# xingyizhou/CenterNet

Hardware: AMD Instinct MI355X
Metric: images/sec whole-node, 512x512 ctdet (higher is better)
Workload: dtype f32s; 1 GPU; ctdet resdcn_18 512x512, batch 32 per GPU (BASELINE configs[1]), network + fused sigmoid/peak-NMS/top-K decode, K=100; global_batch=32, parallelism=image-sharded x1

## Files before the change

centernet_amd/csrc/cn_heads_at.hip:

```cpp
#include "cn_common.h"
#include "cn_internal.h"

namespace {

constexpr int HA_NT = 256;
constexpr int HA_CELLS = 16;
constexpr int HA_CC = 64;
constexpr int HA_ROW = 9 * HA_CC;
constexpr int HA_MAXN = 768;
constexpr int HA_MAXJ = 17;
constexpr int HA_MAXOUT = 2 + 2 * HA_MAXJ + 2;
enum { HA_CTDET = 0, HA_POSE = 1, HA_DDD = 2 };
constexpr int HA_PF = 4;
constexpr int HA_MAXGROUPS = 5;
constexpr int HA_GROUP_HEADS = 3;
constexpr int HA_DDD_OUT = 16;

struct HeadsAtGroup {
    const cn_f32x4 *w1;
    const float *b1, *w2, *b2;
    int n_heads;
    int cout[HA_GROUP_HEADS];
    int col[HA_GROUP_HEADS];
    int voff[HA_GROUP_HEADS];
};

struct HeadsAtArgs {
    const char *feat;
    const float *scores;
    const int32_t *inds, *clses;
    const cn_f32x4 *w1;
    const float *b1;
    const float *w2;
    const float *b2;
    float *dets;
    float *vals;
    float mul;
    int H, W, Cin, pitch, K, hidden, n_heads, N;
    int c0, c1;
    int out;
    int J;
    HeadsAtGroup grp[HA_MAXGROUPS];
    int D;
    int vals_out;
    int raw_depth;
    int half_group;
};

__device__ __forceinline__ void ha_ctdet_row(const HeadsAtArgs &a, size_t row, int ind, const float *o)
{
    float *d = a.dets + row * 6;
    const float score = a.scores[row];
    const float cls = (float)a.clses[row];
    if (ind < 0) {
        const float nan = __builtin_nanf("");
        d[0] = nan; d[1] = nan; d[2] = nan; d[3] = nan; d[4] = score; d[5] = cls;
        if (a.vals)
            for (int v = 0; v < a.out; ++v) a.vals[row * a.out + v] = nan;
        return;
    }
    const int yi = ind / a.W, xi = ind - yi * a.W;
    float xs = (float)xi, ys = (float)yi;
    if (a.n_heads > 1) {
        xs = xs + o[2];
        ys = ys + o[3];
    } else {
        xs = xs + 0.5f;
        ys = ys + 0.5f;
    }
    const float w = o[0];
    const float h = o[1];
    d[0] = xs - w / 2;
    d[1] = ys - h / 2;
    d[2] = xs + w / 2;
    d[3] = ys + h / 2;
    d[4] = score;
    d[5] = cls;
    if (a.vals)
        for (int v = 0; v < a.out; ++v) a.vals[row * a.out + v] = o[v];
}

__device__ __forceinline__ float ha_pose_col(const HeadsAtArgs &a, size_t row, int ind, const float *o, int col)
{
    const int D = 5 + 2 * a.J + 1;
    if (col == 4) return a.scores[row];
    if (col == D - 1) return (float)a.clses[row];
    if (ind < 0) return __builtin_nanf("");
    const int yi = ind / a.W, xi = ind - yi * a.W;
    if (col >= 5) {
        const int v = col - 5;
        return o[2 + v] + (float)((v & 1) ? yi : xi);
    }
    const bool isy = col & 1;
    float c = (float)(isy ? yi : xi);
    if (a.n_heads > 2) c = c + o[2 + 2 * a.J + (isy ? 1 : 0)];
    else c = c + 0.5f;
    const float half = o[isy ? 1 : 0] / 2;
    return col < 2 ? c - half : c + half;
}

template <bool F32S, int CT, int NS, int TASK = HA_CTDET>
__global__ __launch_bounds__(HA_NT) void decode_heads_at_cells_kernel(const HeadsAtArgs a)
{
    constexpr int CG = HA_CELLS / CT;
    constexpr int TPC = HA_NT / CG;
    static_assert(TPC % 64 == 0, "the lanes of a wave read one cell's patch");
    constexpr int HROW = NS * TPC > HA_ROW ? NS * TPC : HA_ROW;
    static_assert(NS * TPC <= HA_MAXN && HA_CELLS * HROW * 4 <= 48 * 1024, "static LDS");
    __shared__ __attribute__((aligned(16))) float lds[HA_CELLS * HROW];
    __shared__ int s_ind[HA_CELLS];
    __shared__ float s_out[HA_CELLS * (TASK == HA_POSE ? HA_MAXOUT : TASK == HA_DDD ? HA_DDD_OUT : 4)];

    const int tid = threadIdx.x;
    const int b = blockIdx.y;
    const int k0 = blockIdx.x * HA_CELLS;
    const int ncell = min(HA_CELLS, a.K - k0);
    const int HW = a.H * a.W;
    int N = a.N, out = a.out, hc0 = a.c0, hc1 = a.c1;
    const cn_f32x4 *w1 = a.w1;
    const float *b1 = a.b1, *w2 = a.w2, *b2 = a.b2;
    if constexpr (TASK == HA_DDD) {
        const HeadsAtGroup &g = a.grp[blockIdx.z];
        N = g.n_heads * a.hidden;
        hc0 = g.cout[0];
        hc1 = g.cout[1];
        out = hc0 + hc1 + g.cout[2];
        w1 = g.w1; b1 = g.b1; w2 = g.w2; b2 = g.b2;
    }

    if (tid < HA_CELLS) {
        int ind = -1;
        if (tid < ncell) {
            ind = a.inds[(size_t)b * a.K + k0 + tid];
            if ((uint32_t)ind >= (uint32_t)HW) ind = -1;
        }
        s_ind[tid] = ind;
    }

    const int nl = tid % TPC, cg = tid / TPC;
    float acc[NS][CT];
#pragma unroll
    for (int s = 0; s < NS; ++s)
#pragma unroll
        for (int i = 0; i < CT; ++i) acc[s][i] = 0.f;

    size_t kq_base = 0;
    for (int c0 = 0; c0 < a.Cin; c0 += HA_CC) {
        const int cc = min(HA_CC, a.Cin - c0);
        const int cq = cc >> 2;
        __syncthreads();
        for (int i = tid; i < HA_CELLS * 9 * cq; i += HA_NT) {
            const int q = i % cq, r = i / cq;
            const int tap = r % 9, cell = r / 9;
            const int ind = s_ind[cell];
            cn_f32x4 v = {0.f, 0.f, 0.f, 0.f};
            if (ind >= 0) {
                const int y = ind / a.W + tap / 3 - 1, x = ind % a.W + tap % 3 - 1;
                if ((unsigned)y < (unsigned)a.H && (unsigned)x < (unsigned)a.W) {
                    const size_t pix = ((size_t)b * a.H + y) * a.W + x;
                    if (F32S) {
                        v = cn_load4_f32s(a.feat, pix, a.pitch, c0 + 4 * q);
                        v *= a.mul;
                    } else {
                        v = *reinterpret_cast<const cn_f32x4 *>(a.feat + (pix * (size_t)a.pitch + c0 + 4 * q) * 4);
                    }
                }
            }
            *reinterpret_cast<cn_f32x4 *>(&lds[cell * HA_ROW + tap * cc + 4 * q]) = v;
        }
        __syncthreads();

        const int nkq = 9 * cq;
        const cn_f32x4 *wq = w1 + kq_base * N;
        cn_f32x4 wn[HA_PF][NS];
#pragma unroll
        for (int p = 0; p < HA_PF; ++p)
#pragma unroll
            for (int s = 0; s < NS; ++s) {
                const int n = nl + s * TPC;
                wn[p][s] = n < N ? wq[(size_t)p * N + n] : cn_f32x4{0.f, 0.f, 0.f, 0.f};
            }
        for (int kq = 0; kq < nkq; kq += HA_PF) {
            cn_f32x4 wv[HA_PF][NS];
#pragma unroll
            for (int p = 0; p < HA_PF; ++p)
#pragma unroll
                for (int s = 0; s < NS; ++s) wv[p][s] = wn[p][s];
            if (kq + HA_PF < nkq) {
#pragma unroll
                for (int p = 0; p < HA_PF; ++p)
#pragma unroll
                    for (int s = 0; s < NS; ++s) {
                        const int n = nl + s * TPC;
                        if (n < N) wn[p][s] = wq[(size_t)(kq + HA_PF + p) * N + n];
                    }
            }
#pragma unroll
            for (int p = 0; p < HA_PF; ++p)
#pragma unroll
                for (int i = 0; i < CT; ++i) {
                    const cn_f32x4 pv = *reinterpret_cast<const cn_f32x4 *>(&lds[(i * CG + cg) * HA_ROW + 4 * (kq + p)]);
#pragma unroll
                    for (int s = 0; s < NS; ++s) {
                        float t = acc[s][i];
                        t = __builtin_fmaf(wv[p][s][0], pv[0], t);
                        t = __builtin_fmaf(wv[p][s][1], pv[1], t);
                        t = __builtin_fmaf(wv[p][s][2], pv[2], t);
                        t = __builtin_fmaf(wv[p][s][3], pv[3], t);
                        acc[s][i] = t;
                    }
                }
        }
        kq_base += (size_t)nkq;
    }

    __syncthreads();
#pragma unroll
    for (int s = 0; s < NS; ++s) {
        const int n = nl + s * TPC;
        if (n < N) {
            const float bias = b1[n];
#pragma unroll
            for (int i = 0; i < CT; ++i)
                lds[(i * CG + cg) * HROW + n] = __builtin_fmaxf(acc[s][i] + bias, 0.f);
        }
    }
    __syncthreads();

    const int nout = HA_CELLS * out;
    for (int o0 = 0; o0 < nout; o0 += HA_NT / 4) {
        const int o = o0 + (tid >> 2), sub = tid & 3;
        const bool live = o < nout;
        const int cell = o / out, r = o - cell * out;
        const int head = (r >= hc0) + (r >= hc0 + hc1);
        float sum = 0.f;
        if (live) {
            const float *w = w2 + (size_t)r * a.hidden;
            const float *h = &lds[cell * HROW + head * a.hidden];
            for (int c = sub; c < a.hidden; c += 4) sum = __builtin_fmaf(w[c], h[c], sum);
        }
        sum += __shfl_xor(sum, 1);
        sum += __shfl_xor(sum, 2);
        if (live && sub == 0) {
            if (b2) sum += b2[r];
            s_out[o] = sum;
        }
    }
    __syncthreads();

    if constexpr (TASK == HA_DDD) {
        const HeadsAtGroup &g = a.grp[blockIdx.z];
        const int D = a.D;
        for (int i = tid; i < ncell * out; i += HA_NT) {
            const int cell = i / out, r = i - cell * out;
            const int head = (r >= hc0) + (r >= hc0 + hc1);
            const int j = r - (head > 0 ? hc0 : 0) - (head > 1 ? hc1 : 0);
            const int col = (head == 0 ? g.col[0] : head == 1 ? g.col[1] : g.col[2]) + j;
            const int vcol = (head == 0 ? g.voff[0] : head == 1 ? g.voff[1] : g.voff[2]) + j;
            const size_t row = (size_t)b * a.K + k0 + cell;
            const int ind = s_ind[cell];
            const float raw = ind < 0 ? __builtin_nanf("") : s_out[i];
            float v = raw;
            if (ind >= 0) {
                if (col < 2) {
                    const int yi = ind / a.W, xi = ind - yi * a.W;
                    v = (float)(col ? yi : xi) + raw;
                } else if (col == 11 && a.raw_depth) {
                    v = 1.0f / (sigmoidf_ref(raw) + 1e-6f) - 1.0f;
                }
            }
            a.dets[row * D + col] = v;
            if (a.vals) a.vals[row * a.vals_out + vcol] = raw;
        }
        if (tid < ncell) {
            const size_t row = (size_t)b * a.K + k0 + tid;
            float *d = a.dets + row * D;
            if (blockIdx.z == 0) {
                d[2] = a.scores[row];
                d[D - 1] = (float)a.clses[row];
            }
            if ((int)blockIdx.z == a.half_group) {
                const int ind = s_ind[tid];
                const int yi = ind / a.W, xi = ind - yi * a.W;
                d[0] = ind < 0 ? __builtin_nanf("") : (float)xi + 0.5f;
                d[1] = ind < 0 ? __builtin_nanf("") : (float)yi + 0.5f;
            }
        }
    } else if (TASK == HA_CTDET) {
        if (tid < ncell) ha_ctdet_row(a, (size_t)b * a.K + k0 + tid, s_ind[tid], &s_out[tid * a.out]);
    } else {
        const int D = 5 + 2 * a.J + 1;
        for (int i = tid; i < ncell * D; i += HA_NT) {
            const int cell = i / D, col = i - cell * D;
            const size_t row = (size_t)b * a.K + k0 + cell;
            a.dets[row * D + col] = ha_pose_col(a, row, s_ind[cell], &s_out[cell * a.out], col);
        }
        if (a.vals)
            for (int i = tid; i < ncell * a.out; i += HA_NT) {
                const int cell = i / a.out;
                a.vals[((size_t)b * a.K + k0) * a.out + i] = s_ind[cell] < 0 ? __builtin_nanf("") : s_out[i];
            }
    }
}

__global__ void decode_pack_cell_w1_kernel(const float *__restrict__ w, float *__restrict__ out, int N, int Cin,
                                           size_t total)
{
    const size_t i = (size_t)blockIdx.x * blockDim.x + threadIdx.x;
    if (i >= total) return;
    const int e = (int)(i & 3);
    const int n = (int)((i >> 2) % N);
    const int k = (int)((i >> 2) / N) * 4 + e;
    const int chunk = k / (9 * HA_CC);
    const int c0 = chunk * HA_CC;
    const int cc = min(HA_CC, Cin - c0);
    const int r = k - chunk * 9 * HA_CC;
    const int tap = r / cc, ci = c0 + r % cc;
    out[i] = w[((size_t)n * Cin + ci) * 9 + tap];
}

}

extern "C" int cn_pack_cell_heads_w1(const float *w, float *out, int N, int Cin, void *stream)
{
    if (!w || !out) return CN_ERR_NULL;
    if (N <= 0 || Cin <= 0) return CN_ERR_SHAPE;
    if (N > HA_MAXN || (N & 63) || (Cin & 31)) return CN_ERR_UNSUPPORTED;
    if (!cn_aligned16(out)) return CN_ERR_ALIGN;
    const size_t total = (size_t)N * Cin * 9;
    hipLaunchKernelGGL(decode_pack_cell_w1_kernel, dim3((unsigned)((total + 255) / 256)), dim3(256), 0,
                       (hipStream_t)stream, w, out, N, Cin, total);
    CN_CHECK_LAUNCH();
    return CN_OK;
}

namespace {

template <int TASK>
void ha_launch(const HeadsAtArgs &a, int N, dim3 grid, bool s, hipStream_t st)
{
    const dim3 block(HA_NT);
#define HA_LAUNCH(CT, NS)                                                                                     \
    do {                                                                                                      \
        if (s) hipLaunchKernelGGL((decode_heads_at_cells_kernel<true, CT, NS, TASK>), grid, block, 0, st, a); \
        else hipLaunchKernelGGL((decode_heads_at_cells_kernel<false, CT, NS, TASK>), grid, block, 0, st, a);  \
    } while (0)
    if (N <= 64) {
        if constexpr (TASK != HA_POSE) HA_LAUNCH(4, 1);
    } else if (N <= 128) HA_LAUNCH(8, 1);
    else if (N <= 256) HA_LAUNCH(16, 1);
    else if (N <= 512) HA_LAUNCH(16, 2);
    else if constexpr (TASK != HA_CTDET) HA_LAUNCH(16, 3);
#undef HA_LAUNCH
}

template <class Limits, class Aligned>
int ha_prepare(HeadsAtArgs &a, const void *feat, int B, int H, int W, int Cin, int pitch, int dtype, float feat_mul,
               const float *scores, const int32_t *inds, const int32_t *clses, int K, int hidden, int n_heads,
               float *dets, float *head_vals, bool ptrs, bool counts, Limits limits, Aligned w1_aligned)
{
    if (!feat || !scores || !inds || !clses || !dets || !ptrs) return CN_ERR_NULL;
    if (B <= 0 || H <= 0 || W <= 0 || Cin <= 0 || K <= 0 || pitch < Cin || !counts) return CN_ERR_SHAPE;
    if (dtype != CN_DTYPE_F32S && dtype != CN_DTYPE_F32) return CN_ERR_UNSUPPORTED;
    if (hidden < 64 || hidden > 256 || (hidden & 63)) return CN_ERR_UNSUPPORTED;
    if (const int rc = limits()) return rc;
    if ((Cin & 31) || (pitch & 3) || (dtype == CN_DTYPE_F32S && (pitch & 31))) return CN_ERR_UNSUPPORTED;
    if ((long)H * W >= (1L << 31) || B > 65535) return CN_ERR_UNSUPPORTED;
    if (!cn_aligned16(feat) || !w1_aligned()) return CN_ERR_ALIGN;
    a.feat = (const char *)feat; a.scores = scores; a.inds = inds; a.clses = clses;
    a.dets = dets; a.vals = head_vals; a.mul = dtype == CN_DTYPE_F32S ? feat_mul : 1.f;
    a.H = H; a.W = W; a.Cin = Cin; a.pitch = pitch; a.K = K; a.hidden = hidden; a.n_heads = n_heads;
    return CN_OK;
}

template <int TASK>
int heads_at_cells(const void *feat, int B, int H, int W, int Cin, int pitch, int dtype, float feat_mul,
                   const float *scores, const int32_t *inds, const int32_t *clses, int K,
                   const float *w1_packed, const float *bias1, int hidden, int n_heads, int J, const float *w2,
                   const float *bias2, float *dets, float *head_vals, void *stream)
{
    constexpr int H0 = TASK == HA_POSE ? 2 : 1;
    HeadsAtArgs a;
    const int rc = ha_prepare(
        a, feat, B, H, W, Cin, pitch, dtype, feat_mul, scores, inds, clses, K, hidden, n_heads, dets, head_vals,
        w1_packed && bias1 && w2, true,
// ... 99 lines not shown
```

centernet_amd/csrc/cn_stem.hip:

```cpp
#include "cn_internal.h"
#include "cn_tuning.h"
#include <type_traits>

namespace {

constexpr int NT = 256;
constexpr int BM = 128;
constexpr int WIN_MAX = 8192;

struct StemArgs {
    const float *x;
    const float *w;
    const float *scale, *shift;
    float *y;
    int H, W, Ho, Wo, Cout, KH, KW, stride, pad, relu, out_pitch, KP, tiles_per_image, cout_pad;
    float x_mul;
    uint32_t *range;
    int y_f32s;
    int stagger;
    int dbg;
};

template <int BN>
__global__ __launch_bounds__(NT) void stem_conv_f32_kernel(const StemArgs a)
// ... 779 lines not shown
                    for (int k = 0; k < 4; ++k) {
                        const st_u32x4 g = *reinterpret_cast<const st_u32x4 *>(strip[k] + lane * 16);
                        *reinterpret_cast<st_u32x4 *>(rowp + lane_off + (unsigned)(8 * k) * (unsigned)pitchB) = g;
                    }
                } else {
                    float *yb = a.y + ((size_t)(b * PH + pr) * PW + (size_t)cb * (BM / 2)) * a.out_pitch + n;
#pragma unroll
                    for (int i = 0; i < MB; ++i)
#pragma unroll
                        for (int q = 0; q < 4; ++q)
#pragma unroll
                            for (int h2 = 0; h2 < 2; ++h2) {
                                const int pc = 2 * (2 * q + lh + 8 * i + 16 * wm) + h2;
                                if (n < a.Cout) yb[(size_t)pc * a.out_pitch] = fmaxf(cur[t][(i * 4 + q) * 2 + h2], hp[i][q][h2]);
                            }
                }
            }
            if (odd) {
#pragma unroll
                for (int e = 0; e < 8 * MB; ++e) cur[t][e] = hp[e >> 3][(e >> 1) & 3][e & 1];
            } else {
#pragma unroll
                for (int e = 0; e < 8 * MB; ++e) cur[t][e] = fmaxf(cur[t][e], hp[e >> 3][(e >> 1) & 3][e & 1]);
            }
        }
        if (!more) break;
        par ^= 1;
        s = ns; y = ny; cb = ncb;
    }
    if (a.range) {
        cn_rng_commit(a.range, 1, rng_bits > 0x7f800000u ? __builtin_inff() : __builtin_bit_cast(float, rng_bits));
        if (a.y_f32s) cn_rng_commit(a.range, 0, rng_out);
    }
}

template <int TPR>
int launch_stem_pool_f32s(const StemArgs &a0, int B, int R, hipStream_t st)
{
    constexpr size_t lds = (size_t)2 * CM_PLANE + (size_t)2 * 64 * SLDW * 2 + 2 * 2 * 64 * 4;
    StemArgs a = a0;
    a.dbg = cn_knobs.stem_dbg & 255;
    a.stagger = cn_knobs.stem_stagger;
    const int nstrips = B * (a.Ho / 2 / R);
    int wgs = nstrips < 512 ? nstrips : 512;
    if (a.stagger == 1000) { wgs = nstrips < 256 ? nstrips : 256; a.stagger = 0; }
    if (a.stagger == 1001) { wgs = nstrips < 768 ? nstrips : 768; a.stagger = 0; }
    if (a.dbg) {
        CN_SET_MAX_LDS_ONCE((stem_pool_f32s_kernel<TPR, true>), lds);
        hipLaunchKernelGGL((stem_pool_f32s_kernel<TPR, true>), dim3(wgs), dim3(NT), lds, st, a, nstrips, R);
    } else {
        CN_SET_MAX_LDS_ONCE((stem_pool_f32s_kernel<TPR, false>), lds);
        hipLaunchKernelGGL((stem_pool_f32s_kernel<TPR, false>), dim3(wgs), dim3(NT), lds, st, a, nstrips, R);
    }
    CN_CHECK_LAUNCH();
    return CN_OK;
}

template <int BN>
int launch_stem_persist_f32s(const StemArgs &a, int B, hipStream_t st)
{
    constexpr size_t lds = (size_t)2 * CM_PLANE + (size_t)2 * BN * SLDW * 2;
    const long total = (long)B * a.tiles_per_image;
    const int wgs = (int)(total < 512 ? total : 512);
    dim3 grid(wgs, cn_cdiv(a.Cout, BN));
    CN_SET_MAX_LDS_ONCE((stem_persist_f32s_kernel<BN>), lds);
    hipLaunchKernelGGL((stem_persist_f32s_kernel<BN>), grid, dim3(NT), lds, st, a, (int)total);
// ... 205 lines not shown

int cn_stem_pool_rows(const ConvCall &c)
{
    if (c.KH != PKH || c.KW != PKW || c.stride != 2 || c.Cout <= 32 || c.Cout > 64) return 0;
    if ((c.cin_pad & 7) || c.cin_pad < PKH * PKW * 3) return 0;
    if (c.Wo % BM || c.Wo / BM > 4 || (c.Ho & 1)) return 0;
    const int PH = c.Ho / 2;
    if (PH % 8 == 0 && (long)c.B * (PH / 8) >= 384) return 8;
    if (PH % 4 == 0 && (long)c.B * (PH / 4) >= 192) return 4;
    return 0;
}

static StemArgs stem_args(const ConvCall &c, bool use_ctl, int tiles_per_image)
{
    StemArgs a = {};
    a.x_mul = (use_ctl && c.ctl && c.ctl->x_mul != 0.f) ? c.ctl->x_mul : 1.f;
    a.range = (use_ctl && c.ctl) ? c.ctl->range : nullptr;
    a.x = (const float *)c.x; a.w = (const float *)c.w; a.scale = c.scale; a.shift = c.shift; a.y = (float *)c.y;
    a.H = c.H; a.W = c.W; a.Ho = c.Ho; a.Wo = c.Wo; a.Cout = c.Cout; a.KH = c.KH; a.KW = c.KW;
    a.stride = c.stride; a.pad = c.pad_h; a.relu = c.relu; a.out_pitch = c.out_pitch; a.KP = c.cin_pad;
    a.tiles_per_image = tiles_per_image;
    a.cout_pad = c.cout_pad;
    return a;
}

int cn_stem_pool_f32s(const ConvCall &c, hipStream_t st)
{
    const int R = cn_stem_pool_rows(c);
    if (!R) return CN_ERR_UNSUPPORTED;
    if (c.stem_y_f32s && ((c.out_pitch & 31) || (((uintptr_t)c.y) & 127u))) return CN_ERR_ALIGN;
    StemArgs a = stem_args(c, true, c.Ho * (c.Wo / BM));
    a.y_f32s = c.stem_y_f32s;
    switch (c.Wo / BM) {
    case 1: return launch_stem_pool_f32s<1>(a, c.B, R, st);
    case 2: return launch_stem_pool_f32s<2>(a, c.B, R, st);
    case 3: return launch_stem_pool_f32s<3>(a, c.B, R, st);
    default: return launch_stem_pool_f32s<4>(a, c.B, R, st);
    }
}

int cn_stem_form(const ConvCall &c, int persistent)
{
    const int KP = c.cin_pad;
    if (KP & 7) return CN_STEM_NONE;
    if (persistent && c.KH == PKH && c.KW == PKW && c.Wo % BM == 0 && (c.stride == 1 || c.stride == 2) &&
        KP >= PKH * PKW * 3) {
        if (c.stem_f32s && c.stride == 2 && c.Cout > 16) return CN_STEM_PERSIST_F32S;
        if (c.stem_f32s && cn_knobs.stem16s && c.stride == 1 && c.Cout <= 16 && c.pad_h == 3 && (c.W & 3) == 0)
            return CN_STEM_16S;
        return CN_STEM_PERSIST;
    }
    int wy, wx;
    if (c.Wo >= BM) {
        wy = c.stride + c.KH;
        wx = (c.Wo - 1) * c.stride + c.KW;
        if (c.Wo % BM == 0) {
            wy = c.KH;
            wx = (BM - 1) * c.stride + c.KW;
        }
    } else {
        const int rows = BM / c.Wo + 2;
        wy = (rows - 1) * c.stride + c.KH;
        wx = (c.Wo - 1) * c.stride + c.KW;
    }
    if ((long)3 * wy * (wx | 1) > WIN_MAX || wx > 2 * NT) return CN_STEM_NONE;
    return CN_STEM_WINDOW;
}

// ... 36 lines not shown
```

Before: 12070 img/s.

## Restructure heads-at-cells decode kernel with weight ring, packed FMA and K-split waves

The per-cell 3x3 head kernel is reorganized so every thread covers all 16 cells, with weights held in a register ring buffer and refilled as they are consumed. LDS patch reads are double-buffered in halves, and accumulation uses packed two-wide FMAs with scheduling barriers. For small hidden widths the reduction dimension is split across the four waves, and their partial sums are combined in LDS. Patch staging now batches its global loads using clamped addresses and masks them afterwards, the second layer unrolls its weight loads, and score and class are prefetched early. The cost is much higher register pressure and more code complexity, since the decode heads are only a small part of the whole network.

Result: no change. 12160 img/s (median of 6 runs) (+0.7%).

```diff
diff --git a/centernet_amd/csrc/cn_heads_at.hip b/centernet_amd/csrc/cn_heads_at.hip
--- a/centernet_amd/csrc/cn_heads_at.hip
+++ b/centernet_amd/csrc/cn_heads_at.hip
@@ -1,5 +1,6 @@
 #include "cn_common.h"
 #include "cn_internal.h"
+#include <type_traits>
 
 namespace {
 
@@ -7,11 +8,12 @@
 constexpr int HA_CELLS = 16;
 constexpr int HA_CC = 64;
 constexpr int HA_ROW = 9 * HA_CC;
+constexpr int HA_SPT = HA_CELLS * HA_ROW / 4 / HA_NT;
 constexpr int HA_MAXN = 768;
 constexpr int HA_MAXJ = 17;
 constexpr int HA_MAXOUT = 2 + 2 * HA_MAXJ + 2;
 enum { HA_CTDET = 0, HA_POSE = 1, HA_DDD = 2 };
-constexpr int HA_PF = 4;
+typedef float ha_f32x2 __attribute__((ext_vector_type(2)));
 constexpr int HA_MAXGROUPS = 5;
 constexpr int HA_GROUP_HEADS = 3;
 constexpr int HA_DDD_OUT = 16;
@@ -47,11 +49,10 @@
     int half_group;
 };
 
-__device__ __forceinline__ void ha_ctdet_row(const HeadsAtArgs &a, size_t row, int ind, const float *o)
+__device__ __forceinline__ void ha_ctdet_row(const HeadsAtArgs &a, size_t row, int ind, const float *o, float score,
+                                             float cls)
 {
     float *d = a.dets + row * 6;
-    const float score = a.scores[row];
-    const float cls = (float)a.clses[row];
     if (ind < 0) {
         const float nan = __builtin_nanf("");
         d[0] = nan; d[1] = nan; d[2] = nan; d[3] = nan; d[4] = score; d[5] = cls;
@@ -99,12 +100,17 @@
     return col < 2 ? c - half : c + half;
 }
 
-template <bool F32S, int CT, int NS, int TASK = HA_CTDET>
+constexpr int ha_ring(int ns, bool ksplit) { return ksplit || ns == 1 ? 9 : ns == 2 ? 6 : 3; }
+
+template <bool F32S, int NS, int TASK = HA_CTDET, bool KSPLIT = false>
 __global__ __launch_bounds__(HA_NT) void decode_heads_at_cells_kernel(const HeadsAtArgs a)
 {
-    constexpr int CG = HA_CELLS / CT;
-    constexpr int TPC = HA_NT / CG;
-    static_assert(TPC % 64 == 0, "the lanes of a wave read one cell's patch");
+    static_assert(!KSPLIT || NS <= 2, "K split: <= 128 channels");
+    constexpr int CT = HA_CELLS;
+    constexpr int TPC = KSPLIT ? 64 : HA_NT;
+    constexpr int R = ha_ring(NS, KSPLIT);
+    static_assert((KSPLIT ? 18 : 72) % R == 0, "a wave's groups of a chunk (18 or 36 / 72 or 144) are whole rounds");
+    static_assert(!KSPLIT || 4 * HA_CELLS * NS * 64 <= HA_CELLS * HA_ROW, "the partial sums fit the patch area");
     constexpr int HROW = NS * TPC > HA_ROW ? NS * TPC : HA_ROW;
     static_assert(NS * TPC <= HA_MAXN && HA_CELLS * HROW * 4 <= 48 * 1024, "static LDS");
     __shared__ __attribute__((aligned(16))) float lds[HA_CELLS * HROW];
@@ -128,101 +134,161 @@
         w1 = g.w1; b1 = g.b1; w2 = g.w2; b2 = g.b2;
     }
 
+    float row_score = 0.f, row_cls = 0.f;
     if (tid < HA_CELLS) {
         int ind = -1;
         if (tid < ncell) {
             ind = a.inds[(size_t)b * a.K + k0 + tid];
             if ((uint32_t)ind >= (uint32_t)HW) ind = -1;
+            if constexpr (TASK == HA_CTDET) {
+                row_score = a.scores[(size_t)b * a.K + k0 + tid];
+                row_cls = (float)a.clses[(size_t)b * a.K + k0 + tid];
+            }
         }
         s_ind[tid] = ind;
     }
 
-    const int nl = tid % TPC, cg = tid / TPC;
-    float acc[NS][CT];
+    constexpr int SB = NS >= 3 ? 1 : HA_SPT;
+    static_assert(HA_SPT % SB == 0, "whole batches");
+    auto stage_patches = [&](int c0, int cc) {
+        const int cq = cc >> 2, total = HA_CELLS * 9 * cq;
+#pragma unroll 1
+        for (int j0 = 0; j0 < HA_SPT; j0 += SB) {
+            cn_f32x4 v[SB];
+#pragma unroll
+            for (int j = 0; j < SB; ++j) {
+                const int i = min(tid + (j0 + j) * HA_NT, total - 1);
+                const int q = i % cq, r = i / cq;
+                const int tap = r % 9, cell = r / 9;
+                const int ind = s_ind[cell], ic = max(ind, 0);
+                const int y = ic / a.W + tap / 3 - 1, x = ic % a.W + tap % 3 - 1;
+                const bool inside = ind >= 0 && (unsigned)y < (unsigned)a.H && (unsigned)x < (unsigned)a.W;
+                const size_t pix = ((size_t)b * a.H + min(max(y, 0), a.H - 1)) * a.W + min(max(x, 0), a.W - 1);
+                if (F32S) {
+                    v[j] = cn_load4_f32s(a.feat, pix, a.pitch, c0 + 4 * q);
+                    v[j] *= a.mul;
+                } else {
+                    v[j] = *reinterpret_cast<const cn_f32x4 *>(a.feat + (pix * (size_t)a.pitch + c0 + 4 * q) * 4);
+                }
+                if (!inside) v[j] = cn_f32x4{0.f, 0.f, 0.f, 0.f};
+            }
+#pragma unroll
+            for (int j = 0; j < SB; ++j) {
+                const int i = tid + (j0 + j) * HA_NT;
+                if (i < total) {
+                    const int q = i % cq, r = i / cq;
+                    *reinterpret_cast<cn_f32x4 *>(&lds[(r / 9) * HA_ROW + (r % 9) * cc + 4 * q]) = v[j];
+                }
+            }
+        }
+    };
+
+    const int nl = tid % TPC;
+    const int wave = __builtin_amdgcn_readfirstlane(tid >> 6);
+    int nc[NS];
+#pragma unroll
+    for (int s = 0; s < NS; ++s) nc[s] = min(nl + s * TPC, N - 1);
+    ha_f32x2 acc[NS][CT];
 #pragma unroll
     for (int s = 0; s < NS; ++s)
 #pragma unroll
-        for (int i = 0; i < CT; ++i) acc[s][i] = 0.f;
-
+        for (int i = 0; i < CT; ++i) acc[s][i] = ha_f32x2{0.f, 0.f};
     size_t kq_base = 0;
     for (int c0 = 0; c0 < a.Cin; c0 += HA_CC) {
         const int cc = min(HA_CC, a.Cin - c0);
-        const int cq = cc >> 2;
+        const int nkq = 9 * (cc >> 2);
+        const int ng = KSPLIT ? nkq >> 2 : nkq;
+        const int kw = KSPLIT ? wave * ng : 0;
+        const cn_f32x4 *wq = w1 + (kq_base + kw) * N;
+        cn_f32x4 ring[R][NS];
+#pragma unroll
+        for (int p = 0; p < R; ++p)
+#pragma unroll
+            for (int s = 0; s < NS; ++s) ring[p][s] = wq[(size_t)p * N + nc[s]];
         __syncthreads();
-        for (int i = tid; i < HA_CELLS * 9 * cq; i += HA_NT) {
-            const int q = i % cq, r = i / cq;
-            const int tap = r % 9, cell = r / 9;
-            const int ind = s_ind[cell];
-            cn_f32x4 v = {0.f, 0.f, 0.f, 0.f};
-            if (ind >= 0) {
-                const int y = ind / a.W + tap / 3 - 1, x = ind % a.W + tap % 3 - 1;
-                if ((unsigned)y < (unsigned)a.H && (unsigned)x < (unsigned)a.W) {
-                    const size_t pix = ((size_t)b * a.H + y) * a.W + x;
-                    if (F32S) {
-                        v = cn_load4_f32s(a.feat, pix, a.pitch, c0 + 4 * q);
-                        v *= a.mul;
-                    } else {
-                        v = *reinterpret_cast<const cn_f32x4 *>(a.feat + (pix * (size_t)a.pitch + c0 + 4 * q) * 4);
-                    }
+        stage_patches(c0, cc);
+        __syncthreads();
+        constexpr int HC = CT / 2;
+        cn_f32x4 pva[HC], pvb[HC];
+        auto read_half = [&](cn_f32x4 (&pv)[HC], int g, int i0) {
+            const float *pp = &lds[4 * (kw + g) + i0 * HA_ROW];
+#pragma unroll
+            for (int i = 0; i < HC; ++i) pv[i] = *reinterpret_cast<const cn_f32x4 *>(pp + i * HA_ROW);
+        };
+        auto fma_half = [&](const cn_f32x4 (&pv)[HC], const cn_f32x4 (&w)[NS], int i0) {
+#pragma unroll
+            for (int e = 0; e < 4; e += 2)
+#pragma unroll
+                for (int i = 0; i < HC; ++i)
+#pragma unroll
+                    for (int s = 0; s < NS; ++s)
+                        acc[s][i0 + i] = __builtin_elementwise_fma(ha_f32x2{w[s][e], w[s][e + 1]},
+                                                                   ha_f32x2{pv[i][e], pv[i][e + 1]}, acc[s][i0 + i]);
+        };
+        auto round = [&](int g0, auto REFILL) {
+            constexpr bool refill = decltype(REFILL)::value;
+#pragma unroll
+            for (int p = 0; p < R; ++p) {
+                read_half(pvb, g0 + p, HC);
+                __builtin_amdgcn_sched_barrier(0);
+                fma_half(pva, ring[p], 0);
+                __builtin_amdgcn_sched_barrier(0);
+                if (refill || p + 1 < R) read_half(pva, g0 + p + 1, 0);
+                __builtin_amdgcn_sched_barrier(0);
+                fma_half(pvb, ring[p], HC);
+                if constexpr (refill) {
+#pragma unroll
+                    for (int s = 0; s < NS; ++s) ring[p][s] = wq[(size_t)(g0 + R + p) * N + nc[s]];
                 }
-            }
-            *reinterpret_cast<cn_f32x4 *>(&lds[cell * HA_ROW + tap * cc + 4 * q]) = v;
-        }
+                __builtin_amdgcn_sched_barrier(0);
+            }
+        };
+        read_half(pva, 0, 0);
+        int g0 = 0;
+        for (; g0 + R < ng; g0 += R) round(g0, std::true_type{});
+        round(g0, std::false_type{});
+        kq_base += (size_t)nkq;
+    }
+
+    if constexpr (KSPLIT) {
+        constexpr int NCH = 64 * NS;
+        constexpr int EPT = HA_CELLS * NCH / HA_NT;
+        float hv[EPT];
+#pragma unroll
+        for (int i = 0; i < EPT; ++i) hv[i] = b1[(tid + HA_NT * i) % NCH];
         __syncthreads();
-
-        const int nkq = 9 * cq;
-        const cn_f32x4 *wq = w1 + kq_base * N;
-        cn_f32x4 wn[HA_PF][NS];
-#pragma unroll
-        for (int p = 0; p < HA_PF; ++p)
-#pragma unroll
-            for (int s = 0; s < NS; ++s) {
-                const int n = nl + s * TPC;
-                wn[p][s] = n < N ? wq[(size_t)p * N + n] : cn_f32x4{0.f, 0.f, 0.f, 0.f};
-            }
-        for (int kq = 0; kq < nkq; kq += HA_PF) {
-            cn_f32x4 wv[HA_PF][NS];
-#pragma unroll
-            for (int p = 0; p < HA_PF; ++p)
-#pragma unroll
-                for (int s = 0; s < NS; ++s) wv[p][s] = wn[p][s];
-            if (kq + HA_PF < nkq) {
-#pragma unroll
-                for (int p = 0; p < HA_PF; ++p)
-#pragma unroll
-                    for (int s = 0; s < NS; ++s) {
-                        const int n = nl + s * TPC;
-                        if (n < N) wn[p][s] = wq[(size_t)(kq + HA_PF + p) * N + n];
-                    }
-            }
-#pragma unroll
-            for (int p = 0; p < HA_PF; ++p)
-#pragma unroll
-                for (int i = 0; i < CT; ++i) {
-                    const cn_f32x4 pv = *reinterpret_cast<const cn_f32x4 *>(&lds[(i * CG + cg) * HA_ROW + 4 * (kq + p)]);
-#pragma unroll
-                    for (int s = 0; s < NS; ++s) {
-                        float t = acc[s][i];
-                        t = __builtin_fmaf(wv[p][s][0], pv[0], t);
-                        t = __builtin_fmaf(wv[p][s][1], pv[1], t);
-                        t = __builtin_fmaf(wv[p][s][2], pv[2], t);
-                        t = __builtin_fmaf(wv[p][s][3], pv[3], t);
-                        acc[s][i] = t;
-                    }
-                }
-        }
-        kq_base += (size_t)nkq;
-    }
-
-    __syncthreads();
-#pragma unroll
-    for (int s = 0; s < NS; ++s) {
-        const int n = nl + s * TPC;
-        if (n < N) {
-            const float bias = b1[n];
-#pragma unroll
-            for (int i = 0; i < CT; ++i)
-                lds[(i * CG + cg) * HROW + n] = __builtin_fmaxf(acc[s][i] + bias, 0.f);
+#pragma unroll
+        for (int s = 0; s < NS; ++s)
+#pragma unroll
+            for (int i = 0; i < CT; ++i) lds[(wave * HA_CELLS + i) * NCH + nl + 64 * s] = acc[s][i][0] + acc[s][i][1];
+        __syncthreads();
+#pragma unroll
+        for (int i = 0; i < EPT; ++i) {
+            const int e = tid + HA_NT * i;
+            float t = lds[e] + lds[HA_CELLS * NCH + e];
+            t = t + lds[2 * HA_CELLS * NCH + e];
+            t = t + lds[3 * HA_CELLS * NCH + e];
+            hv[i] = __builtin_fmaxf(t + hv[i], 0.f);
+        }
+        __syncthreads();
+#pragma unroll
+        for (int i = 0; i < EPT; ++i) {
+            const int e = tid + HA_NT * i;
+            lds[(e / NCH) * HROW + e % NCH] = hv[i];
+        }
+    } else {
+        float bias[NS];
+#pragma unroll
+        for (int s = 0; s < NS; ++s) bias[s] = b1[nc[s]];
+        __syncthreads();
+#pragma unroll
+        for (int s = 0; s < NS; ++s) {
+            const int n = nl + s * TPC;
+            if (n < N) {
+#pragma unroll
+                for (int i = 0; i < CT; ++i)
+                    lds[i * HROW + n] = __builtin_fmaxf(acc[s][i][0] + acc[s][i][1] + bias[s], 0.f);
+            }
         }
     }
     __syncthreads();
@@ -233,16 +299,23 @@
         const bool live = o < nout;
         const int cell = o / out, r = o - cell * out;
         const int head = (r >= hc0) + (r >= hc0 + hc1);
-        float sum = 0.f;
+        float sum = 0.f, bias2 = 0.f;
         if (live) {
             const float *w = w2 + (size_t)r * a.hidden;
             const float *h = &lds[cell * HROW + head * a.hidden];
-            for (int c = sub; c < a.hidden; c += 4) sum = __builtin_fmaf(w[c], h[c], sum);
+            if (b2 && sub == 0) bias2 = b2[r];
+            for (int c = sub; c < a.hidden; c += 64) {
+                float wv[16];
+#pragma unroll
+                for (int u = 0; u < 16; ++u) wv[u] = w[c + 4 * u];
+#pragma unroll
+                for (int u = 0; u < 16; ++u) sum = __builtin_fmaf(wv[u], h[c + 4 * u], sum);
+            }
         }
         sum += __shfl_xor(sum, 1);
         sum += __shfl_xor(sum, 2);
         if (live && sub == 0) {
-            if (b2) sum += b2[r];
+            if (b2) sum += bias2;
             s_out[o] = sum;
         }
     }
@@ -287,7 +360,8 @@
             }
         }
     } else if (TASK == HA_CTDET) {
-        if (tid < ncell) ha_ctdet_row(a, (size_t)b * a.K + k0 + tid, s_ind[tid], &s_out[tid * a.out]);
+        if (tid < ncell)
+            ha_ctdet_row(a, (size_t)b * a.K + k0 + tid, s_ind[tid], &s_out[tid * a.out], row_score, row_cls);
     } else {
         const int D = 5 + 2 * a.J + 1;
         for (int i = tid; i < ncell * D; i += HA_NT) {
@@ -340,17 +414,21 @@
 void ha_launch(const HeadsAtArgs &a, int N, dim3 grid, bool s, hipStream_t st)
 {
     const dim3 block(HA_NT);
-#define HA_LAUNCH(CT, NS)                                                                                     \
+#define HA_LAUNCH(NS, ...)                                                                                      \
     do {                                                                                                      \
-        if (s) hipLaunchKernelGGL((decode_heads_at_cells_kernel<true, CT, NS, TASK>), grid, block, 0, st, a); \
-        else hipLaunchKernelGGL((decode_heads_at_cells_kernel<false, CT, NS, TASK>), grid, block, 0, st, a);  \
+        if (s)                                                                                                \
+            hipLaunchKernelGGL((decode_heads_at_cells_kernel<true, NS, TASK, ##__VA_ARGS__>), grid, block, 0, st, \
+                               a);                                                                            \
+        else                                                                                                  \
+            hipLaunchKernelGGL((decode_heads_at_cells_kernel<false, NS, TASK, ##__VA_ARGS__>), grid, block, 0, st, \
+                               a);                                                                            \
     } while (0)
     if (N <= 64) {
-        if constexpr (TASK != HA_POSE) HA_LAUNCH(4, 1);
-    } else if (N <= 128) HA_LAUNCH(8, 1);
-    else if (N <= 256) HA_LAUNCH(16, 1);
-    else if (N <= 512) HA_LAUNCH(16, 2);
-    else if constexpr (TASK != HA_CTDET) HA_LAUNCH(16, 3);
+        if constexpr (TASK != HA_POSE) HA_LAUNCH(1, true);
+    } else if (N <= 128) HA_LAUNCH(2, true);
+    else if (N <= 256) HA_LAUNCH(1);
+    else if (N <= 512) HA_LAUNCH(2);
+    else if constexpr (TASK != HA_CTDET) HA_LAUNCH(3);
 #undef HA_LAUNCH
 }
 
```

## Add rolling-window stem conv+pool kernel that loads only two new input rows

Applied to the files above, without the earlier changes.

Adds a new fused stem conv+maxpool kernel for one or two 128-wide tiles per row. It keeps a rolling 7-row input window in LDS and fetches only the two new rows per output row, rotating the packed fp16 hi/lo vectors instead of reloading all seven rows. For two tiles per row it runs both tiles in one 512-thread workgroup, sharing the weights and the pool boundary values. Pooled outputs are staged through LDS for coalesced 16-byte stores. This cuts global input traffic and LDS writes, at the cost of extra register shuffles, more LDS per workgroup and possibly lower occupancy.

Measured after the change: 11820 img/s before, 11840 img/s after, median of 3. No clear change (+0.2%).

```diff
diff --git a/centernet_amd/csrc/cn_stem.hip b/centernet_amd/csrc/cn_stem.hip
--- a/centernet_amd/csrc/cn_stem.hip
+++ b/centernet_amd/csrc/cn_stem.hip
@@ -835,6 +835,432 @@
         cn_rng_commit(a.range, 1, rng_bits > 0x7f800000u ? __builtin_inff() : __builtin_bit_cast(float, rng_bits));
         if (a.y_f32s) cn_rng_commit(a.range, 0, rng_out);
     }
+}
+
+template <int ROT>
+__device__ __forceinline__ st_u32x4 cm_rot(st_u32x4 v)
+{
+    return __builtin_shufflevector(v, v, ROT & 3, (ROT + 1) & 3, (ROT + 2) & 3, (ROT + 3) & 3);
+}
+template <int TPR> constexpr int RL_CHUNKS = TPR == 2 ? 4 : 1;
+template <int TPR>
+constexpr size_t RL_LDS = (size_t)TPR * 2 * CM_PLANE + (size_t)2 * 64 * SLDW * 2 + (size_t)2 * TPR * 2 * 64 * 4 +
+                          (size_t)4 * TPR * RL_CHUNKS<TPR> * 1024;
+
+template <int TPR, bool DBG>
+__global__ __launch_bounds__(NT * TPR) void stem_pool_roll_f32s_kernel(const StemArgs a, int nstrips, int R)
+{
+    static_assert(TPR == 1 || TPR == 2, "three and four tiles per row: stem_pool_f32s_kernel");
+    const int dbg = DBG ? (a.dbg & 255) : 0;
+    if (TPR == 1 && a.stagger && blockIdx.x >= 256u) {
+        const unsigned long long t0 = __builtin_readcyclecounter();
+        while (__builtin_readcyclecounter() - t0 < (unsigned long long)a.stagger * 256u) __builtin_amdgcn_s_sleep(32);
+    }
+    constexpr int BN = 64;
+    constexpr int S = 2;
+    constexpr int WN = 2, WM = 2, TM = BM / WM, MB = TM / 32;
+    constexpr int WX = (BM - 1) * S + PKW;
+    constexpr int CHW = RL_CHUNKS<TPR>;
+    constexpr int NTW = NT * TPR;
+    extern __shared__ __attribute__((aligned(16))) char smem[];
+    const int tid = threadIdx.x, team = TPR > 1 ? tid >> 8 : 0, ttid = tid & (NT - 1);
+    const int lane = tid & 63, wave = ttid >> 6;
+    char *winH = smem + team * 2 * CM_PLANE;
+    char *winL = winH + CM_PLANE;
+    _Float16 *WsH = reinterpret_cast<_Float16 *>(smem + TPR * 2 * CM_PLANE);
+    _Float16 *WsL = WsH + BN * SLDW;
+    float *bnd = reinterpret_cast<float *>(WsL + BN * SLDW);
+    char *strip0 = reinterpret_cast<char *>(bnd + 2 * TPR * 2 * BN) + (tid >> 6) * (CHW * 1024);
+
+    const int l31 = lane & 31, lh = lane >> 5;
+    const int wm = wave / WN, wn = wave % WN;
+    const int PH = a.Ho / 2, PW = a.Wo / 2;
+    const int spi = PH / R;
+    const float NEG_INF = -__builtin_huge_valf();
+
+    for (int i = tid; i < TPR * 2 * CM_PLANE / 4; i += NTW) reinterpret_cast<uint32_t *>(smem)[i] = 0u;
+    if (!(dbg & 1 && dbg & 2 && dbg & 4 && dbg & 8 && dbg & 16))
+    for (int i = tid; i < BN * SKP; i += NTW) {
+        const int nrow = i / SKP, k = i - nrow * SKP;
+        const int st = k >> 4, h = (k >> 3) & 1, j = k & 7;
+        const int r = 2 * st + h;
+        const int c = r / PKW, kx = r - c * PKW;
+        const int nn = min(nrow, a.cout_pad - 1);
+        float w = 0.f;
+        if (r < 3 * PKW && j < PKH) w = a.w[(size_t)nn * a.KP + (j * PKW + kx) * 3 + c];
+        const _Float16 hi = (_Float16)w;
+        WsH[nrow * SLDW + k] = hi;
+        WsL[nrow * SLDW + k] = (_Float16)(w - (float)hi);
+    }
+    __syncthreads();
+
+    constexpr int NTAIL = 3 * (WX - NT);
+    const int tt = ttid - 128;
+    const bool tail_thr = tt >= 0 && tt < NTAIL;
+    const int tc = tail_thr ? tt / (WX - NT) : 0, tcol = NT + (tail_thr ? tt % (WX - NT) : 0);
+
+    float v[PROWS], vt[PKH];
+    unsigned vrow = 0;
+    unsigned vcol = 0, vtcol = 0;
+    auto prefetch = [&](int b, int oy, bool full) {
+        const int iy_min = oy * S - a.pad, ix_min = team * BM * S - a.pad;
+        const float *xb = a.x + (size_t)b * 3 * a.H * a.W;
+        const int ix = ix_min + ttid, jx = ix_min + tcol;
+        const bool cok = ix >= 0 && ix < a.W;
+        const bool tok = tail_thr && jx >= 0 && jx < a.W;
+        const int ixc = cok ? ix : 0, jxc = tok ? jx : 0;
+        unsigned mk = 0;
+        if (full) {
+#pragma unroll
+            for (int u = 0; u < PROWS; ++u) {
+                const int c = u / PKH, wy = u % PKH;
+                const int iy = iy_min + wy;
+                const bool rok = iy >= 0 && iy < a.H;
+                const float *rowp = xb + (size_t)(c * a.H + (rok ? iy : 0)) * a.W;
+                v[u] = rowp[ixc];
+                mk |= rok ? (1u << wy) : 0u;
+            }
+            if (tail_thr) {
+#pragma unroll
+                for (int wy = 0; wy < PKH; ++wy) {
+                    const int iy = iy_min + wy;
+                    const bool rok = iy >= 0 && iy < a.H;
+                    vt[wy] = xb[(size_t)(tc * a.H + (rok ? iy : 0)) * a.W + jxc];
+                }
+            }
+        } else {
+#pragma unroll
+            for (int u = 0; u < 6; ++u) {
+                const int c = u >> 1, r = u & 1;
+                const int iy = iy_min + 5 + r;
+                const bool rok = iy >= 0 && iy < a.H;
+                const float *rowp = xb + (size_t)(c * a.H + (rok ? iy : 0)) * a.W;
+                v[u] = rowp[ixc];
+                mk |= rok ? (1u << r) : 0u;
+            }
+            if (tail_thr) {
+#pragma unroll
+                for (int r = 0; r < 2; ++r) {
+                    const int iy = iy_min + 5 + r;
+                    const bool rok = iy >= 0 && iy < a.H;
+                    vt[r] = xb[(size_t)(tc * a.H + (rok ? iy : 0)) * a.W + jxc];
+                }
+            }
+        }
+        vrow = mk;
+        vcol = cok ? 0xffffffffu : 0u;
+        vtcol = tok ? 0xffffffffu : 0u;
+    };
+    uint32_t rng_bits = 0;
+    float rng_out = 0.f;
+    auto prep = [&](float src, uint32_t keep) {
+        const float xs = __builtin_bit_cast(float, __builtin_bit_cast(uint32_t, src) & keep) * a.x_mul;
+        const uint32_t ab = __builtin_bit_cast(uint32_t, xs) & 0x7fffffffu;
+        rng_bits = rng_bits > ab ? rng_bits : ab;
+        return __builtin_amdgcn_fmed3f(xs, -65504.0f, 65504.0f);
+    };
+    auto put7 = [&](int c, int col, const float *src, unsigned cmask, int rot) {
+        float x[8];
+#pragma unroll
+        for (int ky = 0; ky < PKH; ++ky) x[ky] = prep(src[ky], cmask & (((vrow >> ky) & 1u) ? 0xffffffffu : 0u));
+        x[7] = 0.f;
+        st_u32x4 hi, lo;
+#pragma unroll
+        for (int e = 0; e < 4; ++e) {
+            uint32_t h2, l2;
+            cn_split2_bits(x[2 * e], x[2 * e + 1], h2, l2);
+            hi[e] = h2; lo[e] = l2;
+        }
+        if (rot & 1) { hi = cm_rot<3>(hi); lo = cm_rot<3>(lo); }
+        if (rot & 2) { hi = cm_rot<2>(hi); lo = cm_rot<2>(lo); }
+        const int off = c * CM_CH + cm_swz(col) * 16;
+        *reinterpret_cast<st_u32x4 *>(winH + off) = hi;
+        *reinterpret_cast<st_u32x4 *>(winL + off) = lo;
+    };
+    auto put2 = [&](int c, int col, const float *src, unsigned cmask, int o0, int o1) {
+        const float x0 = prep(src[0], cmask & ((vrow & 1u) ? 0xffffffffu : 0u));
+        const float x1 = prep(src[1], cmask & ((vrow & 2u) ? 0xffffffffu : 0u));
+        uint32_t h2, l2;
+        cn_split2_bits(x0, x1, h2, l2);
+        const int off = c * CM_CH + cm_swz(col) * 16;
+        *reinterpret_cast<uint16_t *>(winH + off + o0) = (uint16_t)h2;
+        *reinterpret_cast<uint16_t *>(winH + off + o1) = (uint16_t)(h2 >> 16);
+        *reinterpret_cast<uint16_t *>(winL + off + o0) = (uint16_t)l2;
+        *reinterpret_cast<uint16_t *>(winL + off + o1) = (uint16_t)(l2 >> 16);
+    };
+    auto store_window = [&](int y, bool full) {
+        if (full) {
+#pragma unroll
+            for (int c = 0; c < 3; ++c) put7(c, ttid, v + c * PKH, vcol, y & 3);
+            if (tail_thr) put7(tc, tcol, vt, vtcol, y & 3);
+        } else {
+            const int o0 = ((2 * y + 5) & 7) * 2, o1 = ((2 * y + 6) & 7) * 2;
+#pragma unroll
+            for (int c = 0; c < 3; ++c) put2(c, ttid, v + c * 2, vcol, o0, o1);
+            if (tail_thr) put2(tc, tcol, vt, vtcol, o0, o1);
+        }
+    };
+
+    int aoff[SKS][MB];
+#pragma unroll
+    for (int st = 0; st < SKS; ++st) {
+        const int g = min(2 * st + lh, 3 * PKW - 1);
+        const int c = g / PKW, kx = g - c * PKW;
+#pragma unroll
+        for (int i = 0; i < MB; ++i)
+            aoff[st][i] = c * CM_CH + cm_swz((wm * TM + i * 32 + l31) * S + kx) * 16;
+    }
+    const _Float16 *wH = WsH + (wn * 32 + l31) * SLDW + 8 * lh;
+    const _Float16 *wL = WsL + (wn * 32 + l31) * SLDW + 8 * lh;
+    const int n = wn * 32 + l31;
+    float sc = (a.scale && n < a.Cout) ? a.scale[n] : 1.f;
+    float sf = (a.shift && n < a.Cout) ? a.shift[n] : 0.f;
+    asm volatile("" : "+v"(sc), "+v"(sf));
+
+    auto first_row = [&](int s) { const int p0 = (s % spi) * R; return p0 == 0 ? 0 : 2 * p0 - 1; };
+    int s = blockIdx.x;
+    if (s >= nstrips) return;
+    int y = first_row(s), par = 0;
+    bool full = true;
+    prefetch(s / spi, y, true);
+    float cur[8 * MB];
+    while (true) {
+        const int b = s / spi, p0 = (s % spi) * R;
+        const int ylast = 2 * (p0 + R) - 1;
+        if (y == first_row(s)) {
+#pragma unroll
+            for (int e = 0; e < 8 * MB; ++e) cur[e] = NEG_INF;
+        }
+        if (!(dbg & 2)) store_window(y, full);
+        if (!(dbg & 16)) __syncthreads();
+        int ns = s, ny = y + 1;
+        bool nfull = false;
+        if (ny > ylast) { ns = s + gridDim.x; ny = ns < nstrips ? first_row(ns) : 0; nfull = true; }
+        const bool more = ns < nstrips;
+        if (more && !(dbg & 4)) prefetch(ns / spi, ny, nfull);
+
+        cn_f32x16 acc[MB];
+#pragma unroll
+        for (int i = 0; i < MB; ++i)
+#pragma unroll
+            for (int r = 0; r < 16; ++r) acc[i][r] = 0.f;
+        auto mma = [&](auto rot) {
+            constexpr int ROT = decltype(rot)::value;
+            st_u32x4 fa[2][2][MB];
+            st_f16x8 fb[2][2];
+            auto load_step = [&](int set, int st) {
+#pragma unroll
+                for (int i = 0; i < MB; ++i) {
+                    fa[set][0][i] = cm_rot<ROT>(*reinterpret_cast<const st_u32x4 *>(winH + aoff[st][i]));
+                    fa[set][1][i] = cm_rot<ROT>(*reinterpret_cast<const st_u32x4 *>(winL + aoff[st][i]));
+                }
+                fb[set][0] = *reinterpret_cast<const st_f16x8 *>(wH + 16 * st);
+                fb[set][1] = *reinterpret_cast<const st_f16x8 *>(wL + 16 * st);
+            };
+            if constexpr (ROT != 0) {
+                st_u32x4 raw[2][MB];
+                auto load_raw = [&](int st) {
+#pragma unroll
+                    for (int i = 0; i < MB; ++i) {
+                        raw[0][i] = *reinterpret_cast<const st_u32x4 *>(winH + aoff[st][i]);
+                        raw[1][i] = *reinterpret_cast<const st_u32x4 *>(winL + aoff[st][i]);
+                    }
+                };
+                auto load_fb = [&](int set, int st) {
+                    fb[set][0] = *reinterpret_cast<const st_f16x8 *>(wH + 16 * st);
+                    fb[set][1] = *reinterpret_cast<const st_f16x8 *>(wL + 16 * st);
+                };
+                auto rot_plane = [&](int set, int p) {
+#pragma unroll
+                    for (int i = 0; i < MB; ++i) fa[set][p][i] = cm_rot<ROT>(raw[p][i]);
+                };
+                load_raw(0);
+                load_fb(0, 0);
+                rot_plane(0, 1);
+                rot_plane(0, 0);
+#pragma unroll
+                for (int st = 0; st < SKS; ++st) {
+                    const int cs = st & 1;
+                    const bool next = st + 1 < SKS;
+                    __builtin_amdgcn_sched_barrier(0);
+                    if (next) load_raw(st + 1);
+                    __builtin_amdgcn_sched_barrier(0);
+#pragma unroll
+                    for (int i = 0; i < MB; ++i)
+                        acc[i] = __builtin_amdgcn_mfma_f32_32x32x16_f16(
+                            __builtin_bit_cast(st_f16x8, fa[cs][1][i]), fb[cs][0], acc[i], 0, 0, 0);
+                    __builtin_amdgcn_sched_barrier(0);
+                    if (next) load_fb(cs ^ 1, st + 1);
+                    __builtin_amdgcn_sched_barrier(0);
+#pragma unroll
+                    for (int i = 0; i < MB; ++i)
+                        acc[i] = __builtin_amdgcn_mfma_f32_32x32x16_f16(
+                            __builtin_bit_cast(st_f16x8, fa[cs][0][i]), fb[cs][1], acc[i], 0, 0, 0);
+                    __builtin_amdgcn_sched_barrier(0);
+                    if (next) rot_plane(cs ^ 1, 1);
+                    __builtin_amdgcn_sched_barrier(0);
+#pragma unroll
+                    for (int i = 0; i < MB; ++i)
+                        acc[i] = __builtin_amdgcn_mfma_f32_32x32x16_f16(
+                            __builtin_bit_cast(st_f16x8, fa[cs][0][i]), fb[cs][0], acc[i], 0, 0, 0);
+                    __builtin_amdgcn_sched_barrier(0);
+                    if (next) rot_plane(cs ^ 1, 0);
+                }
+                return;
+            }
+            load_step(0, 0);
+#pragma unroll
+            for (int st = 0; st < SKS; ++st) {
+                const int cs = st & 1;
+                __builtin_amdgcn_sched_barrier(0);
+#pragma unroll
+                for (int i = 0; i < MB; ++i)
+                    acc[i] = __builtin_amdgcn_mfma_f32_32x32x16_f16(
+                        __builtin_bit_cast(st_f16x8, fa[cs][1][i]), fb[cs][0], acc[i], 0, 0, 0);
+                __builtin_amdgcn_sched_barrier(0);
+                if (st + 1 < SKS) load_step(cs ^ 1, st + 1);
+                __builtin_amdgcn_sched_barrier(0);
+#pragma unroll
+                for (int i = 0; i < MB; ++i)
+                    acc[i] = __builtin_amdgcn_mfma_f32_32x32x16_f16(
+                        __builtin_bit_cast(st_f16x8, fa[cs][0][i]), fb[cs][1], acc[i], 0, 0, 0);
+#pragma unroll
+                for (int i = 0; i < MB; ++i)
+                    acc[i] = __builtin_amdgcn_mfma_f32_32x32x16_f16(
+                        __builtin_bit_cast(st_f16x8, fa[cs][0][i]), fb[cs][0], acc[i], 0, 0, 0);
+            }
+        };
+        if (!(dbg & 1)) {
+            switch (y & 3) {
+            case 0: mma(std::integral_constant<int, 0>{}); break;
+            case 1: mma(std::integral_constant<int, 1>{}); break;
+            case 2: mma(std::integral_constant<int, 2>{}); break;
+            default: mma(std::integral_constant<int, 3>{}); break;
+            }
+        }
+
+#pragma unroll
+        for (int i = 0; i < MB; ++i)
+#pragma unroll
+            for (int r = 0; r < 16; ++r) {
+                float t = acc[i][r] * sc + sf;
+                acc[i][r] = a.relu ? fmaxf(t, 0.f) : t;
+            }
+        if (lh == 1) bnd[((par * TPR + team) * 2 + wm) * BN + n] = acc[MB - 1][15];
+        if (!(dbg & 16)) __syncthreads();
+        if (dbg & 8) {
+            if (!more) break;
+            par ^= 1;
+            s = ns; y = ny; full = nfull;
+            continue;
+        }
+        float lastp[MB][4];
+#pragma unroll
+        for (int i = 0; i < MB; ++i)
+#pragma unroll
+            for (int q = 0; q < 4; ++q) lastp[i][q] = __shfl_xor(acc[i][4 * q + 3], 32);
+        float edge = NEG_INF;
+        if (wm == 1) edge = bnd[((par * TPR + team) * 2 + 0) * BN + n];
+        else if (team > 0) edge = bnd[((par * TPR + team - 1) * 2 + 1) * BN + n];
+        float hp[MB][4][2];
+#pragma unroll
+        for (int i = 0; i < MB; ++i)
+#pragma unroll
+            for (int q = 0; q < 4; ++q) {
+                float left;
+                if (lh == 1) left = lastp[i][q];
+                else left = q > 0 ? lastp[i][q - 1] : (i > 0 ? lastp[i - 1][3] : edge);
+                hp[i][q][0] = fmaxf(fmaxf(left, acc[i][4 * q]), acc[i][4 * q + 1]);
+                hp[i][q][1] = fmaxf(fmaxf(acc[i][4 * q + 1], acc[i][4 * q + 2]), acc[i][4 * q + 3]);
+            }
+        const bool odd = (y & 1) != 0;
+        if (odd && y > first_row(s)) {
+            const int pr = (y - 1) >> 1;
+            if (a.y_f32s) {
+                const uint32_t nkeep = n < a.Cout ? 0xffffffffu : 0u;
+                const size_t pitchB = (size_t)a.out_pitch * 4;
+                char *rowp = reinterpret_cast<char *>(a.y) + ((size_t)(b * PH + pr) * PW + (size_t)team * (BM / 2)) * pitchB;
+                const unsigned lane_off = (unsigned)(32 * wm + (lane >> 3)) * (unsigned)pitchB + (unsigned)wn * 128u + (unsigned)(lane & 7) * 16u;
+#pragma unroll
+                for (int k0 = 0; k0 < 4; k0 += CHW) {
+#pragma unroll
+                    for (int k = k0; k < k0 + CHW; ++k)
+#pragma unroll
+                        for (int qq = 0; qq < 2; ++qq) {
+                            const int i = k >> 1, q = 2 * (k & 1) + qq;
+                            float v0 = fmaxf(cur[(i * 4 + q) * 2], hp[i][q][0]);
+                            float v1 = fmaxf(cur[(i * 4 + q) * 2 + 1], hp[i][q][1]);
+                            cn_rng_upd1(rng_out, v0);
+                            cn_rng_upd1(rng_out, v1);
+                            uint32_t hb, lb;
+                            cn_split2_bits(__builtin_amdgcn_fmed3f(v0, -65504.0f, 65504.0f),
+                                           __builtin_amdgcn_fmed3f(v1, -65504.0f, 65504.0f), hb, lb);
+                            hb &= nkeep;
+                            lb &= nkeep;
+                            char *dst = strip0 + (k % CHW) * 1024 + (4 * qq + 2 * lh) * 128 + l31 * 2;
+                            *reinterpret_cast<uint16_t *>(dst) = (uint16_t)hb;
+                            *reinterpret_cast<uint16_t *>(dst + 64) = (uint16_t)lb;
+                            *reinterpret_cast<uint16_t *>(dst + 128) = (uint16_t)(hb >> 16);
+                            *reinterpret_cast<uint16_t *>(dst + 192) = (uint16_t)(lb >> 16);
+                        }
+#pragma unroll
+                    for (int k = k0; k < k0 + CHW; ++k) {
+                        const st_u32x4 g = *reinterpret_cast<const st_u32x4 *>(strip0 + (k % CHW) * 1024 + lane * 16);
+                        *reinterpret_cast<st_u32x4 *>(rowp + lane_off + (unsigned)(8 * k) * (unsigned)pitchB) = g;
+                    }
+                }
+            } else {
+                float *yb = a.y + ((size_t)(b * PH + pr) * PW + (size_t)team * (BM / 2)) * a.out_pitch + n;
+#pragma unroll
+                for (int i = 0; i < MB; ++i)
+#pragma unroll
+                    for (int q = 0; q < 4; ++q)
+#pragma unroll
+                        for (int h2 = 0; h2 < 2; ++h2) {
+                            const int pc = 2 * (2 * q + lh + 8 * i + 16 * wm) + h2;
+                            if (n < a.Cout) yb[(size_t)pc * a.out_pitch] = fmaxf(cur[(i * 4 + q) * 2 + h2], hp[i][q][h2]);
+                        }
+            }
+        }
+        if (odd) {
+#pragma unroll
+            for (int e = 0; e < 8 * MB; ++e) cur[e] = hp[e >> 3][(e >> 1) & 3][e & 1];
+        } else {
+#pragma unroll
+            for (int e = 0; e < 8 * MB; ++e) cur[e] = fmaxf(cur[e], hp[e >> 3][(e >> 1) & 3][e & 1]);
+        }
+        if (!more) break;
+        par ^= 1;
+        s = ns; y = ny; full = nfull;
+    }
+    if (a.range) {
+        cn_rng_commit(a.range, 1, rng_bits > 0x7f800000u ? __builtin_inff() : __builtin_bit_cast(float, rng_bits));
+        if (a.y_f32s) cn_rng_commit(a.range, 0, rng_out);
+    }
+}
+
+template <int TPR>
+int launch_stem_pool_roll_f32s(const StemArgs &a0, int B, int R, hipStream_t st)
+{
+    constexpr size_t lds = RL_LDS<TPR>;
+    static_assert(lds * (TPR == 1 ? 2 : 1) <= 160 * 1024, "LDS budget");
+    StemArgs a = a0;
+    a.dbg = cn_knobs.stem_dbg & 255;
+    a.stagger = TPR == 1 ? cn_knobs.stem_stagger : 0;
+    const int nstrips = B * (a.Ho / 2 / R);
+    const int resident = TPR == 1 ? 512 : 256;
+    int wgs = nstrips < resident ? nstrips : resident;
+    if (a.stagger == 1000) { wgs = nstrips < 256 ? nstrips : 256; a.stagger = 0; }
+    if (a.stagger == 1001) { wgs = nstrips < 768 ? nstrips : 768; a.stagger = 0; }
+    if (a.dbg) {
+        CN_SET_MAX_LDS_ONCE((stem_pool_roll_f32s_kernel<TPR, true>), lds);
+        hipLaunchKernelGGL((stem_pool_roll_f32s_kernel<TPR, true>), dim3(wgs), dim3(NT * TPR), lds, st, a, nstrips, R);
+    } else {
+        CN_SET_MAX_LDS_ONCE((stem_pool_roll_f32s_kernel<TPR, false>), lds);
+        hipLaunchKernelGGL((stem_pool_roll_f32s_kernel<TPR, false>), dim3(wgs), dim3(NT * TPR), lds, st, a, nstrips, R);
+    }
+    CN_CHECK_LAUNCH();
+    return CN_OK;
 }
 
 template <int TPR>
@@ -1106,8 +1532,8 @@
     StemArgs a = stem_args(c, true, c.Ho * (c.Wo / BM));
     a.y_f32s = c.stem_y_f32s;
     switch (c.Wo / BM) {
-    case 1: return launch_stem_pool_f32s<1>(a, c.B, R, st);
-    case 2: return launch_stem_pool_f32s<2>(a, c.B, R, st);
+    case 1: return launch_stem_pool_roll_f32s<1>(a, c.B, R, st);
+    case 2: return launch_stem_pool_roll_f32s<2>(a, c.B, R, st);
     case 3: return launch_stem_pool_f32s<3>(a, c.B, R, st);
     default: return launch_stem_pool_f32s<4>(a, c.B, R, st);
     }
```
